# PrimeIntellect-ai/protocol

Measured on AMD Instinct MI355X. Metric: task x worker pair-evals/sec (full-swarm match), higher is better.
Workload: dtype u64

## Files before the change

protocol_amd/csrc/pm_device.h:

```cpp
#ifndef PM_DEVICE_H
#define PM_DEVICE_H

#include <hip/hip_runtime.h>
#include <stdint.h>

#include "pm_engine.h"

namespace pm {

static constexpr double PM_RAD = 3.14159265358979323846 / 180.0;
static constexpr uint64_t PM_KEY_NOLOC = 0x7FEFFFFFFFFFFFFFull;
static constexpr double PM_A_MAX_SAFE = 1.0 - 1.0 / 1048576.0;
static constexpr double PM_A_CHORD_MIN = 1.3e-6;
static constexpr uint32_t PM_CARVE_SLOTS = 8192;
static constexpr uint32_t PM_CARVE_PART = 64;
static constexpr uint32_t PM_CARVE_SEL_CAP = 256;
static constexpr uint32_t PM_CARVE_SLOT_BITS = 13;
static constexpr uint32_t PM_CARVE_BIG_SLOTS = 262144;
static constexpr uint32_t PM_CARVE_SLOT_BITS_BIG = 18;
static constexpr uint32_t PM_CARVE_SLOT_BITS_MEM = 21;
static constexpr double PM_TIE_BAND = 1.0 / 68719476736.0;
static constexpr double PM_TIE_BAND_BIG = 1.0 / 2147483648.0;
static constexpr double PM_TIE_BAND_MEM = 1.0 / 268435456.0;
static constexpr uint32_t PM_PROP_ROW = 96;
// ... 85 lines not shown
  const uint32_t* t_prefix;
  pm_assignment* table;
  uint32_t* task_col;
  pm_assignment* h_table;
  uint32_t* h_gtask;
};

struct MatchPrepArgs {
  uint32_t W, G;
  const int32_t* group_of;
  const uint32_t *g_cfg, *g_n, *g_off, *members, *addr_rank, *g_task;
  uint64_t* sel;
  uint32_t *first, *count;
  uint32_t *rank_in_group, *by_rank;
  uint32_t* g_task_next;
};

struct RowUpdateArgs {
  uint32_t n;
  const double *lat_in, *lon_in;
  const uint32_t* u32_in;
  uint32_t *flags, *gpu_count, *gpu_mem, *gpu_cls, *cpu_cores, *ram, *storage, *addr_rank, *site;
  double *lat, *lon, *coslat;
  double *ux, *uy, *uz;
};

enum { CARVE_MODE_FORM = 0, CARVE_MODE_MERGE = 1 };
enum { CARVE_STATE_RUNNING = 0, CARVE_STATE_DONE = 1, CARVE_STATE_UNCERTAIN = 2, CARVE_STATE_OVERFLOW = 3,
       CARVE_STATE_ABORTED = 4 };
enum {
// ... 143 lines not shown
void launch_explain(const CompatArgs& p, const uint32_t* rows, uint32_t n, uint32_t stride, uint32_t* why_out, hipStream_t s);
void launch_config_report(const ReportArgs& a, uint32_t max_blocks, hipStream_t s);
void launch_task_report(const ReportArgs& a, uint32_t max_blocks, hipStream_t s);
void launch_geo(const double* lat, const double* lon, double* coslat, double* ux, double* uy, double* uz, uint32_t W,
                hipStream_t s);
void launch_triad(const double* b, const double* c, double* a, size_t n, hipStream_t s);
#ifdef PM_ROW_BENCH
hipError_t launch_row_bench(const CarveArgs* d_args, uint32_t seed, uint32_t ci, uint32_t reps, uint32_t mode, unsigned long long* d_out, hipStream_t s);
#endif
void launch_row_network_test(const uint64_t* keys, const uint32_t* sites, uint32_t n_waves, uint32_t n_per_wave, uint32_t slot_bits,
                             uint64_t ulps, uint32_t upto, uint64_t* rows_out, uint32_t* mismatches, hipStream_t s);
static constexpr uint32_t PM_DK_WORDS = 20;
void launch_distance_key_test(const double* in, const double* geo, uint32_t n, uint32_t mode, double* out, hipStream_t s);
void launch_update_rows(const RowUpdateArgs& a, hipStream_t s);
void launch_worker_selector(const int32_t* group_of, const uint32_t* g_cfg, uint32_t R, const uint32_t* rows,
                            uint64_t* sel, hipStream_t s);
void launch_eligible_selector(const uint32_t* wflags, const int32_t* group_of, const uint64_t* compat,
                              uint64_t enabled, uint32_t W, const uint8_t* shard, uint32_t my_rank, uint64_t* sel,
                              hipStream_t s);
void launch_chooser_rank(const int32_t* group_of, const uint64_t* g_id, const uint32_t* count, uint32_t R,
                         const uint32_t* rows, uint64_t seed, uint32_t* rank, hipStream_t s);
void launch_table_scatter(const pm_assignment* x, const uint32_t* xrow, uint32_t W, pm_assignment* table,
                          uint32_t* task_col, uint32_t* g_task_next, const uint64_t* t_live, const uint32_t* t_prefix,
                          hipStream_t s);
void launch_group_rank(const int32_t* group_of, const uint32_t* g_n, const uint32_t* g_off, const uint32_t* members,
                       const uint32_t* addr_rank, uint32_t W, uint32_t* rank_in_group, uint32_t* by_rank,
                       hipStream_t s);
void launch_claim_publish(const ClaimArgs& a, hipStream_t s);
void launch_match_prep(const MatchPrepArgs& a, hipStream_t s);
void launch_build_planes(const uint64_t* col_mask, uint32_t n_cols, uint32_t c_begin, uint32_t c_end, uint32_t stride,
                         uint32_t n_planes, uint64_t* planes, hipStream_t s);
void launch_pair_sweep(int variant, const uint64_t* row_sel, uint32_t R, const uint64_t* col_mask,
                       const uint64_t* planes, uint32_t c_begin, uint32_t c_end, uint32_t stride, uint32_t n_planes,
                       uint32_t* first, uint32_t* count, hipStream_t s, bool inited = false);
void launch_pair_select(int variant, const uint64_t* row_sel, uint32_t R, const uint64_t* col_mask,
                        const uint64_t* planes, uint32_t c_begin, uint32_t c_end, uint32_t stride, uint32_t n_planes,
                        const uint32_t* rank, uint32_t* out, hipStream_t s);
void launch_task_prefix(const uint64_t* live, uint32_t w_begin, uint32_t w_end, uint32_t* prefix, hipStream_t s);
void launch_task_delete(const uint32_t* slots, uint32_t n, uint64_t* tmask, uint64_t* live, uint64_t* planes,
                        uint32_t stride, uint32_t n_planes, hipStream_t s);
void launch_task_intern(const uint64_t* tmask, const uint64_t* live, uint32_t u_begin, uint32_t u_end, uint64_t valid,
                        uint64_t* keys, uint32_t n_slots, uint32_t* vals, uint32_t* counter_and_overflow, uint64_t* umask,
                        uint32_t cap_u, hipStream_t s);
void launch_task_compact_class(const uint32_t* first_c, const uint32_t* count_c, const uint64_t* tmask, uint64_t valid,
// ... 26 lines not shown
```

protocol_amd/csrc/pm_engine.cpp:

```cpp
#include <hip/hip_runtime.h>

#include <algorithm>
#include <atomic>
#include <cmath>
#include <chrono>
#include <cstdio>
#include <cstdlib>
#include <cstring>
#include <functional>
#include <memory>
#include <mutex>
#include <string>
#include <thread>
#include <unordered_map>
#include <vector>

#include "pm_device.h"
#include "pm_engine.h"
#include "pm_internal.h"
#include "pm_members.h"

namespace pm {

static thread_local std::string g_last_error;
// ... 123 lines not shown
  *out = e;
  return PM_OK;
}

void pm_engine_destroy(pm_engine* e) {
  if (!e) return;
  (void)hipSetDevice(e->cfg.device);
  (void)hipStreamSynchronize(e->stream);
  e->d_cfgs.release(); e->d_alts.release(); e->d_model_bits.release();
  e->d_flags.release(); e->d_gpu_count.release(); e->d_gpu_mem.release(); e->d_gpu_cls.release();
  e->d_cpu_cores.release(); e->d_ram.release(); e->d_storage.release(); e->d_addr_rank.release();
  e->d_lat.release(); e->d_lon.release(); e->d_coslat.release(); e->d_compat.release();
  e->d_ux.release(); e->d_uy.release(); e->d_uz.release();
  for (int k = 0; k < 3; ++k) { e->d_c_u[k].release(); e->d_cc_u[k].release(); }
  e->d_tmask.release(); e->d_tplanes.release(); e->d_created.release(); e->d_tlive.release(); e->d_tprefix.release();
  e->d_first_c.release(); e->d_count_c.release(); e->d_tdel.release();
  e->d_group_of.release(); e->d_g_cfg.release(); e->d_g_n.release(); e->d_g_off.release();
  e->d_g_task.release(); e->d_g_task_next.release(); e->d_members.release(); e->d_by_rank.release();
  e->d_rank_in_group.release(); e->d_g_id.release();
  e->d_order.release(); e->d_c_lat.release(); e->d_c_lon.release(); e->d_c_cos.release();
  e->d_cc_lat.release(); e->d_cc_lon.release(); e->d_cc_cos.release(); e->d_slot_pos.release(); e->d_slot_wid.release();
  e->d_site.release(); e->d_c_site.release(); e->d_cc_site.release(); e->d_prop.release(); e->d_prop_send.release(); e->d_seed_map.release(); e->d_seed_prefix.release(); e->d_seed_slots.release(); e->d_prep_block_counts.release(); e->d_prep_counts.release();
  e->d_c_compat.release(); e->d_keys.release(); e->d_bits.release(); e->d_status.release(); e->d_carve_args.release();
  e->d_m_cfg.release(); e->d_m_n.release(); e->d_m_off.release(); e->d_m_members.release();
  e->d_cfgbits.release(); e->d_stream_sq.release(); e->d_stream_row_lo.release(); e->d_stream_row_hi.release();
  e->d_stream_ctl.release(); e->d_stream_trace.release();
  e->d_sel.release(); e->d_wplanes.release(); e->d_sel_perm.release();
  e->d_first.release(); e->d_count.release(); e->d_rank.release(); e->d_chosen.release(); e->d_perm.release();
  e->d_table.release(); e->d_task_col.release(); e->d_shard.release(); e->d_own_rows.release(); e->d_xrow.release();
  e->d_sel_own.release(); e->d_table_x.release(); e->d_row_stage.release(); if (e->h_row_pin) (void)hipHostFree(e->h_row_pin); if (e->ev_row_stage) (void)hipEventDestroy(e->ev_row_stage); e->d_nb_idx.release(); e->d_nb_val.release();
  if (e->h_gstage) (void)hipHostFree(e->h_gstage);
// ... 39 lines not shown
  }
  std::lock_guard<std::mutex> lk(e->mu);
  if (e->dist_phase != 0) return set_error(PM_ESTATE, "a stepwise tick is in progress");
  HIPCHK(hipSetDevice(e->cfg.device));
  e->cfgs.assign(cfgs, cfgs + n_cfgs);
  e->alts.assign(alts, alts + n_alts);
  int32_t rc = upload(e->d_cfgs, e->cfgs.data(), e->cfgs.size(), e->stream);
  if (rc) return rc;
  rc = upload(e->d_alts, e->alts.data(), e->alts.size(), e->stream);
  if (rc) return rc;
  HIPCHK(e->d_model_bits.ensure(1));
  HIPCHK(hipStreamSynchronize(e->stream));
  e->have_cfgs = true;
  e->compat_dirty = true;
  e->tplanes_dirty = true;
  return PM_OK;
}

int32_t pm_set_model_table(pm_engine* e, const uint32_t* bits, uint32_t n_rows, uint32_t n_classes) {
  if (!e || (n_rows && n_classes && !bits)) return set_error(PM_EINVAL, "null argument");
  std::lock_guard<std::mutex> lk(e->mu);
  HIPCHK(hipSetDevice(e->cfg.device));
  const size_t words = size_t(n_rows) * ((n_classes + 31u) / 32u);
  e->model_bits.assign(bits, bits + words);
  e->model_rows = n_rows;
  e->model_classes = n_classes;
  e->cls_check_dirty = true;
  int32_t rc = upload(e->d_model_bits, e->model_bits.data(), words, e->stream);
  if (rc) return rc;
  HIPCHK(hipStreamSynchronize(e->stream));
// ... 22 lines not shown
```

protocol_amd/csrc/pm_engine_match.inc:

```

static int32_t ensure_task_planes(pm_engine* e) {
  if (!e->have_tasks) return set_error(PM_ESTATE, "tasks must be uploaded first");
  const uint32_t n_planes = uint32_t(e->cfgs.size());
  const uint32_t stride = e->t_cap / 64u;
  if (e->tplanes_dirty) {
    HIPCHK(e->d_tplanes.ensure(std::max<size_t>(size_t(stride) * (n_planes + 1), 1)));
    launch_build_planes(e->d_tmask.p, e->t_cap, e->t_lo, e->t_cap, stride, n_planes, e->d_tplanes.p, e->stream);
    HIPCHK(hipGetLastError());
    e->tplanes_dirty = false;
  }
  if (e->tprefix_dirty) {
    launch_task_prefix(e->d_tlive.p, e->t_lo / 64u, stride, e->d_tprefix.p, e->stream);
    HIPCHK(hipGetLastError());
    e->tprefix_dirty = false;
  }
  return PM_OK;
}

static uint32_t task_position(pm_engine* e, uint32_t u) {
  if (u == PM_NONE || u < e->t_lo || u >= e->t_cap) return PM_NONE;
  if (!e->h_tprefix_valid) {
    const uint32_t stride = e->t_cap / 64u;
    e->h_tprefix.assign(stride, 0);
    uint32_t acc = 0;
    for (uint32_t j = e->t_lo / 64u; j < stride; ++j) {
      e->h_tprefix[j] = acc;
      acc += uint32_t(__builtin_popcountll(e->h_tlive[j]));
    }
    e->h_tprefix_valid = true;
// ... 55 lines not shown
  rc = ensure_task_planes(e);
  if (rc) return rc;
  host_mark("match: task planes");
  const uint32_t R = dist ? uint32_t(e->h_own_rows.size()) : e->W;
  const uint32_t* rows = dist ? e->d_own_rows.p : nullptr;
  rc = ensure_sweep_outputs(e, R);
  if (rc) return rc;
  HIPCHK(e->d_sel.ensure(std::max<uint32_t>(e->W, 1)));
  HIPCHK(e->d_table.ensure(std::max<uint32_t>(e->W, 1)));
  HIPCHK(e->d_task_col.ensure(std::max<uint32_t>(e->W, 1)));
  if (e->W == 0) return PM_OK;
  const uint32_t n_planes = uint32_t(e->cfgs.size());

  host_mark("match: selector launch");
  const size_t G = G_ub ? G_ub : e->d_n_groups;
  if (!dist) {
    MatchPrepArgs m{};
    m.W = e->W;
    m.G = uint32_t(G);
    m.group_of = e->d_group_of.p;
    m.g_cfg = e->d_g_cfg.p;
    m.g_n = e->d_g_n.p;
    m.g_off = e->d_g_off.p;
    m.members = e->d_members.p;
    m.addr_rank = e->d_addr_rank.p;
    m.g_task = e->d_g_task.p;
    m.sel = e->d_sel.p;
    m.first = e->d_first.p;
    m.count = e->d_count.p;
    m.rank_in_group = e->d_rank_in_group.p;
    m.by_rank = e->d_by_rank.p;
    m.g_task_next = e->d_g_task_next.p;
    launch_match_prep(m, e->stream);
  } else {
    launch_worker_selector(e->d_group_of.p, e->d_g_cfg.p, R, rows, e->d_sel.p, e->stream);
  }
  const bool time_sweep = e->cfg.time_proposer != 0;
  if (time_sweep) HIPCHK(hipEventRecord(e->kev[4], e->stream));
  const uint32_t t_stride = e->t_cap / 64u;
  launch_pair_sweep(variant, e->d_sel.p, R, e->d_tmask.p, e->d_tplanes.p, e->t_lo, e->t_cap, t_stride, n_planes,
                    e->d_first.p, e->d_count.p, e->stream, !dist);
  if (time_sweep) HIPCHK(hipEventRecord(e->kev[5], e->stream));
  e->k_sweep_recorded = time_sweep;
  const uint32_t* chosen = e->d_first.p;
  if (e->cfg.chooser == PM_CHOOSE_SEEDED) {
    launch_chooser_rank(e->d_group_of.p, e->d_g_id.p, e->d_count.p, R, rows, e->cfg.chooser_seed, e->d_rank.p,
                        e->stream);
    launch_pair_select(variant, e->d_sel.p, R, e->d_tmask.p, e->d_tplanes.p, e->t_lo, e->t_cap, t_stride, n_planes,
                       e->d_rank.p, e->d_chosen.p, e->stream);
    chosen = e->d_chosen.p;
  }
  if (dist) {
    launch_group_rank(e->d_group_of.p, e->d_g_n.p, e->d_g_off.p, e->d_members.p, e->d_addr_rank.p, e->W,
                      e->d_rank_in_group.p, e->d_by_rank.p, e->stream);
    if (G) HIPCHK(hipMemcpyAsync(e->d_g_task_next.p, e->d_g_task.p, G * 4, hipMemcpyDeviceToDevice, e->stream));
  }
  ClaimArgs c{};
  c.R = R;
  c.rows = rows;
  c.group_of = e->d_group_of.p;
  c.g_n = e->d_g_n.p;
  c.g_off = e->d_g_off.p;
  c.g_task = e->d_g_task.p;
  c.g_id = e->d_g_id.p;
  c.g_task_next = e->d_g_task_next.p;
  c.chosen = chosen;
  c.rank_in_group = e->d_rank_in_group.p;
  c.by_rank = e->d_by_rank.p;
  c.t_live = e->d_tlive.p;
  c.t_prefix = e->d_tprefix.p;
  c.table = dist ? e->d_table_x.p + size_t(e->dist_rank) * e->dist_cap_t : e->d_table.p;
  c.task_col = e->d_task_col.p;
  c.h_table = claim_h_table;
  c.h_gtask = claim_h_gtask;
  launch_claim_publish(c, e->stream);
  HIPCHK(hipGetLastError());
  if (want_count && count_out) {
    count_out->resize(R);
    HIPCHK(hipMemcpyAsync(count_out->data(), e->d_count.p, size_t(R) * 4, hipMemcpyDeviceToHost, e->stream));
  }
  return PM_OK;
}

static int32_t pub_buffer(pm_engine* e, PubTable& t, uint32_t rows, uint64_t** out) {
  uint64_t* words = t.words.load(std::memory_order_relaxed);
  if (t.cap_rows < rows || !words) {
    const size_t cap = std::max<size_t>(size_t(rows) + rows / 8 + 64, 64);
    uint64_t* nw = nullptr;
    if (hipHostMalloc((void**)&nw, cap * 32) != hipSuccess || !nw)
      return set_error(PM_ENOMEM, "out of pinned host memory for the published table");
    std::memset(nw, 0, cap * 32);
// ... 205 lines not shown
```

protocol_amd/csrc/pm_engine_state.inc:

```
struct pm_engine {
  pm_engine_config cfg{};
  hipStream_t stream = nullptr;
  hipStream_t stream_owned = nullptr;
  bool own_stream = true;
  hipEvent_t ev[6]{};
  hipEvent_t kev[6]{};
  hipEvent_t k_carve_begin = nullptr;
  hipEvent_t k_compat_end = nullptr;
  bool one_event_behind_carve = false;
  float k_ms_compat = 0, k_ms_carve = 0, k_ms_sweep = 0;
  bool k_sweep_recorded = false, k_compat_recorded = false;
  std::chrono::steady_clock::time_point tick_t0{};
  bool end_event_queued = false;
  uint64_t tick_cand_sum = 0;
  unsigned long long carve_prof[64]{};
  unsigned long long carve_why[24]{};
  uint32_t debug_mem_above = 0;
  uint32_t debug_abort_after = 0;
  uint32_t delta_pushes = 0;
  uint32_t merge_streamed = 0;
  uint32_t merge_stream_min = 512;
  uint32_t prune_mode = 1;
  uint32_t prune_factor = 512;
  uint32_t walk_cap_div = 0;
// ... 43 lines not shown
  uint32_t t_regrowths = 0, t_compactions = 0;
  bool have_tasks = false;
  std::vector<uint64_t> h_tmask, h_tuid, h_tlive;
  std::vector<int64_t> h_created;
  std::vector<uint32_t> h_tprefix;
  bool h_tprefix_valid = false;
  bool tasks_have_uid = false;
  std::unordered_map<uint64_t, uint32_t> uid_to_u;
  bool uid_map_valid = false;
  uint32_t cfg_app_count[PM_MAX_CONFIGS]{};
  bool cfg_app_valid = false;
  DevBuf<uint64_t> d_tmask, d_tplanes, d_tlive;
  DevBuf<int64_t> d_created;
  DevBuf<uint32_t> d_tprefix, d_first_c, d_count_c, d_tdel;
  bool tplanes_dirty = true, tprefix_dirty = true;

  std::vector<Group> groups;
  size_t n_dead_groups = 0;
  bool flags_dirty = false;
  std::vector<int32_t> h_group_of;
  uint64_t id_rng = 0;
  bool groups_dirty = true;
  bool groups_delta_ok = false;
  std::vector<uint32_t> delta_free;
  uint32_t delta_tail_from = PM_NONE;
  bool flags_delta_ok = false;
  std::vector<uint32_t> delta_flags;
  uint32_t* h_delta_pin[2] = {nullptr, nullptr};
  size_t h_delta_cap[2] = {0, 0};
  DevBuf<uint32_t> d_delta[2];
// ... 83 lines not shown
```

protocol_amd/csrc/pm_engine_tasks.inc:

```
static int32_t tasks_alloc(pm_engine* e, uint32_t cap) {
  e->h_tmask.assign(cap, 0);
  e->h_created.assign(cap, 0);
  e->h_tlive.assign(cap / 64u, 0);
  if (e->tasks_have_uid) e->h_tuid.assign(cap, 0); else e->h_tuid.clear();
  e->t_cap = cap;
  e->t_lo = cap;
  e->T = e->t_dead = 0;
  e->h_tprefix_valid = false;
  HIPCHK(e->d_tmask.ensure(cap));
  HIPCHK(e->d_created.ensure(cap));
  HIPCHK(e->d_tlive.ensure(cap / 64u));
  HIPCHK(e->d_tprefix.ensure(cap / 64u));
  HIPCHK(hipMemsetAsync(e->d_tmask.p, 0, size_t(cap) * 8, e->stream));
  HIPCHK(hipMemsetAsync(e->d_tlive.p, 0, size_t(cap / 64u) * 8, e->stream));
  e->tplanes_dirty = true;
  e->tprefix_dirty = true;
  return PM_OK;
}

static int32_t tasks_push_range(pm_engine* e, uint32_t u0, uint32_t u1) {
  if (u1 <= u0) return PM_OK;
  const uint32_t w0 = u0 / 64u, w1 = (u1 + 63u) / 64u;
  HIPCHK(hipMemcpyAsync(e->d_tmask.p + u0, e->h_tmask.data() + u0, size_t(u1 - u0) * 8, hipMemcpyHostToDevice, e->stream));
  HIPCHK(hipMemcpyAsync(e->d_created.p + u0, e->h_created.data() + u0, size_t(u1 - u0) * 8, hipMemcpyHostToDevice, e->stream));
  HIPCHK(hipMemcpyAsync(e->d_tlive.p + w0, e->h_tlive.data() + w0, size_t(w1 - w0) * 8, hipMemcpyHostToDevice, e->stream));
  return PM_OK;
}

static constexpr uint32_t PM_TASK_DEAD_SLACK = 4096;

static int32_t tasks_rebuild(pm_engine* e, uint32_t cap) {
// ... 62 lines not shown
  for (uint32_t u = clear_from; u < lo; ++u) e->h_tmask[u] = 0;
  for (uint32_t w = clear_from / 64u; w < cap / 64u; ++w) e->h_tlive[w] = 0;
  std::memcpy(e->h_tmask.data() + lo, t->topo_mask, size_t(n) * 8);
  std::memcpy(e->h_created.data() + lo, t->created_at, size_t(n) * 8);
  if (t->uid) std::memcpy(e->h_tuid.data() + lo, t->uid, size_t(n) * 8);
  for (uint32_t u = lo; u < cap; ++u) e->h_tlive[u >> 6] |= 1ull << (u & 63u);
  e->t_lo = lo;
  e->T = n;
  e->t_dead = 0;
  e->h_tprefix_valid = false;
  rc = tasks_push_range(e, clear_from, cap);
  if (rc) return rc;
  HIPCHK(hipStreamSynchronize(e->stream));
  e->tplanes_dirty = true;
  e->tprefix_dirty = true;
  e->have_tasks = true;
  size_t n_claim = 0;
  for (const Group& g : e->groups) n_claim += (!g.dead && g.task != PM_NONE);
  if (n_claim) {
    size_t hcap = 64;
    while (hcap < n_claim * 4) hcap <<= 1;
    const uint64_t EMPTY = ~0ull;
    std::vector<uint64_t> keys(hcap, EMPTY);
    std::vector<uint32_t> vals(hcap, PM_NONE);
    auto slot_of = [&](uint64_t k) {
      size_t h = size_t(splitmix64_mix(k)) & (hcap - 1);
      while (keys[h] != EMPTY && keys[h] != k) h = (h + 1) & (hcap - 1);
      return h;
    };
    if (e->tasks_have_uid) {
// ... 97 lines not shown
      }
    }
  }
  {
    int32_t rcp = tasks_push_range(e, lo, e->t_lo);
    if (rcp) return rcp;
  }
  if (!e->tplanes_dirty && e->d_tplanes.p)
    launch_build_planes(e->d_tmask.p, e->t_cap, lo, e->t_lo, e->t_cap / 64u, uint32_t(e->cfgs.size()), e->d_tplanes.p,
                        e->stream);
  HIPCHK(hipGetLastError());
  HIPCHK(hipStreamSynchronize(e->stream));
  e->t_lo = lo;
  e->T += n;
  e->tprefix_dirty = true;
  e->h_tprefix_valid = false;
  pub_shift_tasks(e, n);
  return PM_OK;
}

int32_t pm_tasks_delete(pm_engine* e, const uint64_t* uids, uint32_t n, uint32_t* n_deleted) {
  if (!e || (n && !uids)) return set_error(PM_EINVAL, "null argument");
  std::lock_guard<std::mutex> lk(e->mu);
  HIPCHK(hipSetDevice(e->cfg.device));
  if (n_deleted) *n_deleted = 0;
  if (!e->have_tasks) return set_error(PM_ESTATE, "tasks must be uploaded first");
  if (!e->tasks_have_uid) return set_error(PM_ESTATE, "the task table carries no ids (pm_task_soa.uid)");
  if (e->dist_phase != 0) return set_error(PM_ESTATE, "a stepwise tick is in progress");
  ABSORB_PENDING(e);
  if (!e->uid_map_valid) {
// ... 35 lines not shown
    e->h_tlive[u >> 6] &= ~(1ull << (u & 63u));
  }
  e->h_tprefix_valid = false;
  for (size_t g = 0; g < e->groups.size(); ++g) {
    const Group& gr = e->groups[g];
    if (!gr.dead && gr.task != PM_NONE && std::binary_search(slots.begin(), slots.end(), gr.task))
      dissolve_locked(e, uint32_t(g));
  }
  e->T -= uint32_t(slots.size());
  e->t_dead += uint32_t(slots.size());
  while (e->t_lo < e->t_cap && !((e->h_tlive[e->t_lo >> 6] >> (e->t_lo & 63u)) & 1ull)) {
    e->t_lo++;
    e->t_dead--;
  }
  e->tprefix_dirty = true;
  e->h_tprefix_valid = false;
  if (e->t_dead > e->T + PM_TASK_DEAD_SLACK) {
    int32_t rc = tasks_rebuild(e, e->t_cap);
    if (rc) return rc;
    e->t_compactions++;
  }
  if (n_deleted) *n_deleted = uint32_t(slots.size());
  pub_patch(e, nullptr);
  return PM_OK;
}
```

protocol_amd/csrc/pm_kernels.hip:

```cpp
#include <hip/hip_runtime.h>
#include <stdint.h>

#include "pm_device.h"

#if defined(__HIP_DEVICE_COMPILE__) && !defined(__gfx950__)
#error "pm_kernels.hip is written for gfx950 (MI355X): see the note on the placement kernels' fences above"
#endif

namespace pm {


template <int CTRL, int ROW_MASK>
__device__ __forceinline__ uint32_t dpp_add_step(uint32_t v) {
  return v + (uint32_t)__builtin_amdgcn_update_dpp(0, (int)v, CTRL, ROW_MASK, 0xF, false);
}
__device__ __forceinline__ uint32_t wave_incl_scan_u32(uint32_t v) {
  v = dpp_add_step<0x111, 0xF>(v);
  v = dpp_add_step<0x112, 0xF>(v);
  v = dpp_add_step<0x114, 0xF>(v);
  v = dpp_add_step<0x118, 0xF>(v);
  v = dpp_add_step<0x142, 0xA>(v);
  v = dpp_add_step<0x143, 0xC>(v);
  return v;
}
// ... 338 lines not shown
  out[r] = res;
}

__global__ __launch_bounds__(64) void task_prefix_kernel(const uint64_t* __restrict__ live, uint32_t w_begin,
                                                         uint32_t w_end, uint32_t* __restrict__ prefix) {
  const uint32_t lane = threadIdx.x;
  uint32_t acc = 0;
  for (uint32_t j0 = w_begin; j0 < w_end; j0 += 64u) {
    const uint32_t j = j0 + lane;
    const uint32_t cnt = j < w_end ? (uint32_t)__popcll(live[j]) : 0u;
    const uint32_t incl = wave_incl_scan_u32(cnt);
    if (j < w_end) prefix[j] = acc + incl - cnt;
    acc += __shfl(incl, 63, 64);
  }
}
__global__ __launch_bounds__(256) void task_delete_kernel(const uint32_t* __restrict__ slots, uint32_t n,
                                                          uint64_t* __restrict__ tmask,
                                                          uint64_t* __restrict__ live, uint64_t* __restrict__ planes,
                                                          uint32_t stride, uint32_t n_planes) {
  const uint32_t k = blockIdx.x * 256u + threadIdx.x;
  if (k >= n) return;
  const uint32_t u = slots[k];
  const uint64_t bit = 1ull << (u & 63u);
  tmask[u] = 0ull;
  atomicAnd((unsigned long long*)&live[u >> 6], ~bit);
  for (uint32_t b = 0; b <= n_planes; ++b)
    atomicAnd((unsigned long long*)&planes[(size_t)b * stride + (u >> 6)], ~bit);
}
__global__ __launch_bounds__(256) void task_compact_kernel(const uint32_t* __restrict__ first_u,
                                                           const uint32_t* __restrict__ count_u, uint32_t u_begin,
// ... 70 lines not shown
  uint32_t first = PM_NONE, count = 0u;
  if (m != 0ull) {
    uint32_t h = (uint32_t)splitmix64_mix(m) & h_mask;
    while (keys[h] != m) h = (h + 1u) & h_mask;
    const uint32_t id = vals[h];
    first = first_c[id];
    count = count_c[id];
  }
  first_out[pos] = first;
  count_out[pos] = count;
}

__global__ __launch_bounds__(256) void worker_selector_kernel(const int32_t* __restrict__ group_of,
                                                              const uint32_t* __restrict__ g_cfg, uint32_t R,
                                                              const uint32_t* __restrict__ rows,
                                                              uint64_t* __restrict__ sel) {
  const uint32_t r = blockIdx.x * 256u + threadIdx.x;
  if (r >= R) return;
  const int32_t g = group_of[rows ? rows[r] : r];
  sel[r] = g >= 0 ? (1ull << g_cfg[g]) : 0ull;
}

__global__ __launch_bounds__(256) void chooser_rank_kernel(const int32_t* __restrict__ group_of,
                                                           const uint64_t* __restrict__ g_id,
                                                           const uint32_t* __restrict__ count, uint32_t R,
                                                           const uint32_t* __restrict__ rows, uint64_t seed,
                                                           uint32_t* __restrict__ rank) {
  const uint32_t r = blockIdx.x * 256u + threadIdx.x;
  if (r >= R) return;
  const int32_t g = group_of[rows ? rows[r] : r];
  const uint32_t n = count[r];
  rank[r] = (g >= 0 && n) ? (uint32_t)(splitmix64_mix(seed ^ g_id[g]) % n) : PM_NONE;
}

__global__ __launch_bounds__(256) void eligible_selector_kernel(const uint32_t* __restrict__ wflags,
// ... 29 lines not shown
  by_rank[off + idx] = w;
}

__global__ __launch_bounds__(256) void match_prep_kernel(MatchPrepArgs p) {
  const uint32_t w = blockIdx.x * 256u + threadIdx.x;
  if (w < p.G) p.g_task_next[w] = p.g_task[w];
  if (w >= p.W) return;
  const int32_t g = p.group_of[w];
  p.first[w] = PM_NONE;
  p.count[w] = 0u;
  if (g < 0) {
    p.sel[w] = 0ull;
    p.rank_in_group[w] = 0;
    return;
  }
  p.sel[w] = 1ull << p.g_cfg[g];
  const uint32_t n = p.g_n[g], off = p.g_off[g], my = p.addr_rank[w];
  uint32_t idx = 0;
  for (uint32_t k = 0; k < n; ++k) idx += p.addr_rank[p.members[off + k]] < my;
  p.rank_in_group[w] = idx;
  p.by_rank[off + idx] = w;
}

__device__ __forceinline__ uint32_t task_position(const uint64_t* __restrict__ live, const uint32_t* __restrict__ prefix,
                                                  uint32_t u) {
  return prefix[u >> 6] + (uint32_t)__popcll(live[u >> 6] & ((1ull << (u & 63u)) - 1ull));
}

__global__ __launch_bounds__(256) void claim_publish_kernel(ClaimArgs p) {
  const uint32_t r = blockIdx.x * 256u + threadIdx.x;
  const bool in = r < p.R;
// ... 33 lines not shown
  }
  if (p.h_table) {
    static_assert(sizeof(pm_assignment) == 32, "a row is two 16-byte pieces");
    __shared__ uint4 s_rows[512];
    s_rows[2u * threadIdx.x] = make_uint4(a.task, a.group_slot, a.group_index, a.group_size);
    s_rows[2u * threadIdx.x + 1u] = make_uint4(a.next_worker, 0u, (uint32_t)a.group_id, (uint32_t)(a.group_id >> 32));
    if (g >= 0 && a.group_index == 0u) p.h_gtask[g] = t;
    __syncthreads();
    const uint32_t row0 = blockIdx.x * 256u;
    const uint32_t n16 = 2u * (p.R - row0 < 256u ? p.R - row0 : 256u);
    uint4* const dst = reinterpret_cast<uint4*>(p.h_table + row0);
    for (uint32_t k = threadIdx.x; k < n16; k += 256u) dst[k] = s_rows[k];
  }
}

__global__ __launch_bounds__(256) void table_scatter_kernel(const pm_assignment* __restrict__ x,
                                                            const uint32_t* __restrict__ xrow, uint32_t W,
                                                            pm_assignment* __restrict__ table,
                                                            uint32_t* __restrict__ task_col,
                                                            uint32_t* __restrict__ g_task_next,
                                                            const uint64_t* __restrict__ t_live,
                                                            const uint32_t* __restrict__ t_prefix) {
  const uint32_t w = blockIdx.x * 256u + threadIdx.x;
  if (w >= W) return;
  pm_assignment a = x[xrow[w]];
  if (a.group_slot != PM_NONE && a.task != PM_NONE) g_task_next[a.group_slot] = a.task;
  if (a.task != PM_NONE) a.task = task_position(t_live, t_prefix, a.task);
  table[w] = a;
  task_col[w] = a.task;
}
// ... 57 lines not shown
```

protocol_amd/csrc/pm_launch.inc:

```

void launch_compat(const CompatArgs& a, hipStream_t s) {
  if (a.W == 0) return;
  if (a.W < 65536u)
    hipLaunchKernelGGL(compat_sliced_kernel, dim3((a.W + 63u) / 64u), dim3(256), 0, s, a);
  else
    hipLaunchKernelGGL(compat_kernel, dim3((a.W + 255u) / 256u), dim3(256), 0, s, a);
}
void launch_triad(const double* b, const double* c, double* a, size_t n, hipStream_t s) {
  hipLaunchKernelGGL(triad_kernel, dim3(256 * 32), dim3(256), 0, s, b, c, a, n);
}
void launch_row_network_test(const uint64_t* keys, const uint32_t* sites, uint32_t n_waves, uint32_t n_per_wave, uint32_t slot_bits,
                             uint64_t ulps, uint32_t upto, uint64_t* rows_out, uint32_t* mismatches, hipStream_t s) {
  hipLaunchKernelGGL(row_network_test_kernel, dim3(n_waves / 4u), dim3(256), 0, s, keys, sites, n_per_wave, slot_bits, ulps, upto, rows_out,
                     mismatches);
}
void launch_distance_key_test(const double* in, const double* geo, uint32_t n, uint32_t mode, double* out, hipStream_t s) {
  if (n == 0) return;
  hipLaunchKernelGGL(distance_key_test_kernel, dim3((n + 255u) / 256u), dim3(256), 0, s, in, geo, n, mode, out);
}
void launch_geo(const double* lat, const double* lon, double* coslat, double* ux, double* uy, double* uz, uint32_t W,
                hipStream_t s) {
  if (W == 0) return;
  hipLaunchKernelGGL(geo_kernel, dim3((W + 255u) / 256u), dim3(256), 0, s, lat, lon, coslat, ux, uy, uz, W);
}
void launch_update_rows(const RowUpdateArgs& a, hipStream_t s) {
  if (a.n == 0) return;
  hipLaunchKernelGGL(update_rows_kernel, dim3((a.n + 255u) / 256u), dim3(256), 0, s, a);
}
void launch_worker_selector(const int32_t* group_of, const uint32_t* g_cfg, uint32_t R, const uint32_t* rows,
                            uint64_t* sel, hipStream_t s) {
  if (R == 0) return;
  hipLaunchKernelGGL(worker_selector_kernel, dim3((R + 255u) / 256u), dim3(256), 0, s, group_of, g_cfg, R, rows, sel);
}
void launch_chooser_rank(const int32_t* group_of, const uint64_t* g_id, const uint32_t* count, uint32_t R,
                         const uint32_t* rows, uint64_t seed, uint32_t* rank, hipStream_t s) {
  if (R == 0) return;
  hipLaunchKernelGGL(chooser_rank_kernel, dim3((R + 255u) / 256u), dim3(256), 0, s, group_of, g_id, count, R, rows,
                     seed, rank);
}
void launch_eligible_selector(const uint32_t* wflags, const int32_t* group_of, const uint64_t* compat,
                              uint64_t enabled, uint32_t W, const uint8_t* shard, uint32_t my_rank, uint64_t* sel,
                              hipStream_t s) {
  if (W == 0) return;
  hipLaunchKernelGGL(eligible_selector_kernel, dim3((W + 255u) / 256u), dim3(256), 0, s, wflags, group_of, compat,
                     enabled, W, shard, my_rank, sel);
}
void launch_table_scatter(const pm_assignment* x, const uint32_t* xrow, uint32_t W, pm_assignment* table,
// ... 2 lines not shown
  if (W == 0) return;
  hipLaunchKernelGGL(table_scatter_kernel, dim3((W + 255u) / 256u), dim3(256), 0, s, x, xrow, W, table, task_col,
                     g_task_next, t_live, t_prefix);
}
void launch_group_rank(const int32_t* group_of, const uint32_t* g_n, const uint32_t* g_off, const uint32_t* members,
                       const uint32_t* addr_rank, uint32_t W, uint32_t* rank_in_group, uint32_t* by_rank,
                       hipStream_t s) {
  if (W == 0) return;
  hipLaunchKernelGGL(group_rank_kernel, dim3((W + 255u) / 256u), dim3(256), 0, s, group_of, g_n, g_off, members,
                     addr_rank, W, rank_in_group, by_rank);
}
void launch_match_prep(const MatchPrepArgs& a, hipStream_t s) {
  const uint32_t n = a.W > a.G ? a.W : a.G;
  if (n == 0) return;
  hipLaunchKernelGGL(match_prep_kernel, dim3((n + 255u) / 256u), dim3(256), 0, s, a);
}
void launch_claim_publish(const ClaimArgs& a, hipStream_t s) {
  if (a.R == 0) return;
  hipLaunchKernelGGL(claim_publish_kernel, dim3((a.R + 255u) / 256u), dim3(256), 0, s, a);
}

void launch_build_planes(const uint64_t* col_mask, uint32_t n_cols, uint32_t c_begin, uint32_t c_end, uint32_t stride,
                         uint32_t n_planes, uint64_t* planes, hipStream_t s) {
  const uint32_t w0 = c_begin / 64u, w1 = (c_end + 63u) / 64u;
  if (w1 <= w0) return;
  hipLaunchKernelGGL(build_planes_kernel, dim3(((w1 - w0) * 64u + 255u) / 256u), dim3(256), 0, s, col_mask, n_cols, w0,
                     w1, stride, n_planes, planes);
}

void launch_pair_sweep(int variant, const uint64_t* row_sel, uint32_t R, const uint64_t* col_mask,
// ... 213 lines not shown
```

Measured before the change: 1048 billion.

## Precompute per-config task summaries and fuse match prep with claim publish

Adds a plane-summary kernel that computes, for each config plane, the first eligible task and the count of eligible tasks. It is recomputed only when the task set changes. Because each worker's selector is a single config bit, the per-worker pair sweep reduces to a table lookup and is skipped for non-legacy variants. In the non-distributed, unseeded case, a new fused match_publish kernel replaces the prep, sweep and claim kernels, cutting launches and redundant passes. The risks are extra invalidation bookkeeping (tsum_dirty) and a possible semantic mismatch if selectors ever carry more than one config bit.

```diff
diff --git a/protocol_amd/csrc/pm_device.h b/protocol_amd/csrc/pm_device.h
--- a/protocol_amd/csrc/pm_device.h
+++ b/protocol_amd/csrc/pm_device.h
@@ -123,6 +123,24 @@
   uint32_t *first, *count;
   uint32_t *rank_in_group, *by_rank;
   uint32_t* g_task_next;
+  const uint32_t *tsum_first, *tsum_count;
+};
+
+struct MatchPublishArgs {
+  uint32_t W, G;
+  uint32_t members_cap;
+  const int32_t* group_of;
+  const uint32_t *g_cfg, *g_n, *g_off, *members, *addr_rank, *g_task;
+  const uint64_t* g_id;
+  const uint32_t *tsum_first, *tsum_count;
+  const uint64_t* t_live;
+  const uint32_t* t_prefix;
+  uint32_t* g_task_next;
+  uint32_t* count_out;
+  pm_assignment* table;
+  uint32_t* task_col;
+  pm_assignment* h_table;
+  uint32_t* h_gtask;
 };
 
 struct RowUpdateArgs {
@@ -296,7 +314,8 @@
 void launch_distance_key_test(const double* in, const double* geo, uint32_t n, uint32_t mode, double* out, hipStream_t s);
 void launch_update_rows(const RowUpdateArgs& a, hipStream_t s);
 void launch_worker_selector(const int32_t* group_of, const uint32_t* g_cfg, uint32_t R, const uint32_t* rows,
-                            uint64_t* sel, hipStream_t s);
+                            uint64_t* sel, const uint32_t* tsum_first, const uint32_t* tsum_count, uint32_t* first,
+                            uint32_t* count, hipStream_t s);
 void launch_eligible_selector(const uint32_t* wflags, const int32_t* group_of, const uint64_t* compat,
                               uint64_t enabled, uint32_t W, const uint8_t* shard, uint32_t my_rank, uint64_t* sel,
                               hipStream_t s);
@@ -310,6 +329,9 @@
                        hipStream_t s);
 void launch_claim_publish(const ClaimArgs& a, hipStream_t s);
 void launch_match_prep(const MatchPrepArgs& a, hipStream_t s);
+void launch_match_publish(const MatchPublishArgs& a, hipStream_t s);
+void launch_plane_summary(const uint64_t* planes, uint32_t stride, uint32_t w_begin, uint32_t w_end, uint32_t n_planes,
+                          uint32_t* tsum_first, uint32_t* tsum_count, hipStream_t s);
 void launch_build_planes(const uint64_t* col_mask, uint32_t n_cols, uint32_t c_begin, uint32_t c_end, uint32_t stride,
                          uint32_t n_planes, uint64_t* planes, hipStream_t s);
 void launch_pair_sweep(int variant, const uint64_t* row_sel, uint32_t R, const uint64_t* col_mask,
diff --git a/protocol_amd/csrc/pm_engine.cpp b/protocol_amd/csrc/pm_engine.cpp
--- a/protocol_amd/csrc/pm_engine.cpp
+++ b/protocol_amd/csrc/pm_engine.cpp
@@ -161,7 +161,7 @@
   e->d_ux.release(); e->d_uy.release(); e->d_uz.release();
   for (int k = 0; k < 3; ++k) { e->d_c_u[k].release(); e->d_cc_u[k].release(); }
   e->d_tmask.release(); e->d_tplanes.release(); e->d_created.release(); e->d_tlive.release(); e->d_tprefix.release();
-  e->d_first_c.release(); e->d_count_c.release(); e->d_tdel.release();
+  e->d_first_c.release(); e->d_count_c.release(); e->d_tdel.release(); e->d_tsum.release();
   e->d_group_of.release(); e->d_g_cfg.release(); e->d_g_n.release(); e->d_g_off.release();
   e->d_g_task.release(); e->d_g_task_next.release(); e->d_members.release(); e->d_by_rank.release();
   e->d_rank_in_group.release(); e->d_g_id.release();
@@ -231,6 +231,7 @@
   e->have_cfgs = true;
   e->compat_dirty = true;
   e->tplanes_dirty = true;
+  e->tsum_dirty = true;
   return PM_OK;
 }
 
diff --git a/protocol_amd/csrc/pm_engine_match.inc b/protocol_amd/csrc/pm_engine_match.inc
--- a/protocol_amd/csrc/pm_engine_match.inc
+++ b/protocol_amd/csrc/pm_engine_match.inc
@@ -8,11 +8,25 @@
     launch_build_planes(e->d_tmask.p, e->t_cap, e->t_lo, e->t_cap, stride, n_planes, e->d_tplanes.p, e->stream);
     HIPCHK(hipGetLastError());
     e->tplanes_dirty = false;
+    e->tsum_dirty = true;
   }
   if (e->tprefix_dirty) {
     launch_task_prefix(e->d_tlive.p, e->t_lo / 64u, stride, e->d_tprefix.p, e->stream);
     HIPCHK(hipGetLastError());
     e->tprefix_dirty = false;
+  }
+  if (e->tsum_dirty) {
+    HIPCHK(e->d_tsum.ensure(2u * PM_MAX_CONFIGS));
+    const bool timed = e->cfg.time_proposer != 0 && e->cfg.sweep_variant != 1u;
+    if (timed) HIPCHK(hipEventRecord(e->kev[4], e->stream));
+    launch_plane_summary(e->d_tplanes.p, stride, e->t_lo / 64u, stride, n_planes, e->d_tsum.p, e->d_tsum.p + PM_MAX_CONFIGS,
+                         e->stream);
+    HIPCHK(hipGetLastError());
+    if (timed) {
+      HIPCHK(hipEventRecord(e->kev[5], e->stream));
+      e->k_sweep_recorded = true;
+    }
+    e->tsum_dirty = false;
   }
   return PM_OK;
 }
@@ -98,10 +112,14 @@
 
   host_mark("match: selector launch");
   const size_t G = G_ub ? G_ub : e->d_n_groups;
-  if (!dist) {
-    MatchPrepArgs m{};
+  const bool summary = variant != 1;
+  const uint32_t* const tsum_first = summary ? e->d_tsum.p : nullptr;
+  const uint32_t* const tsum_count = summary ? e->d_tsum.p + PM_MAX_CONFIGS : nullptr;
+  if (summary && !dist && e->cfg.chooser != PM_CHOOSE_SEEDED) {
+    MatchPublishArgs m{};
     m.W = e->W;
-    m.G = uint32_t(G);
+    m.G = uint32_t(std::min(G, std::min(e->d_g_cfg.cap, std::min(e->d_g_n.cap, e->d_g_off.cap))));
+    m.members_cap = uint32_t(std::min<size_t>(e->d_members.cap, 0xFFFFFFFFu));
     m.group_of = e->d_group_of.p;
     m.g_cfg = e->d_g_cfg.p;
     m.g_n = e->d_g_n.p;
@@ -109,56 +127,87 @@
     m.members = e->d_members.p;
     m.addr_rank = e->d_addr_rank.p;
     m.g_task = e->d_g_task.p;
-    m.sel = e->d_sel.p;
-    m.first = e->d_first.p;
-    m.count = e->d_count.p;
-    m.rank_in_group = e->d_rank_in_group.p;
-    m.by_rank = e->d_by_rank.p;
+    m.g_id = e->d_g_id.p;
+    m.tsum_first = tsum_first;
+    m.tsum_count = tsum_count;
+    m.t_live = e->d_tlive.p;
+    m.t_prefix = e->d_tprefix.p;
     m.g_task_next = e->d_g_task_next.p;
-    launch_match_prep(m, e->stream);
+    m.count_out = want_count && count_out ? e->d_count.p : nullptr;
+    m.table = e->d_table.p;
+    m.task_col = e->d_task_col.p;
+    m.h_table = claim_h_table;
+    m.h_gtask = claim_h_gtask;
+    launch_match_publish(m, e->stream);
+    HIPCHK(hipGetLastError());
   } else {
-    launch_worker_selector(e->d_group_of.p, e->d_g_cfg.p, R, rows, e->d_sel.p, e->stream);
-  }
-  const bool time_sweep = e->cfg.time_proposer != 0;
-  if (time_sweep) HIPCHK(hipEventRecord(e->kev[4], e->stream));
-  const uint32_t t_stride = e->t_cap / 64u;
-  launch_pair_sweep(variant, e->d_sel.p, R, e->d_tmask.p, e->d_tplanes.p, e->t_lo, e->t_cap, t_stride, n_planes,
-                    e->d_first.p, e->d_count.p, e->stream, !dist);
-  if (time_sweep) HIPCHK(hipEventRecord(e->kev[5], e->stream));
-  e->k_sweep_recorded = time_sweep;
-  const uint32_t* chosen = e->d_first.p;
-  if (e->cfg.chooser == PM_CHOOSE_SEEDED) {
-    launch_chooser_rank(e->d_group_of.p, e->d_g_id.p, e->d_count.p, R, rows, e->cfg.chooser_seed, e->d_rank.p,
-                        e->stream);
-    launch_pair_select(variant, e->d_sel.p, R, e->d_tmask.p, e->d_tplanes.p, e->t_lo, e->t_cap, t_stride, n_planes,
-                       e->d_rank.p, e->d_chosen.p, e->stream);
-    chosen = e->d_chosen.p;
-  }
-  if (dist) {
-    launch_group_rank(e->d_group_of.p, e->d_g_n.p, e->d_g_off.p, e->d_members.p, e->d_addr_rank.p, e->W,
-                      e->d_rank_in_group.p, e->d_by_rank.p, e->stream);
-    if (G) HIPCHK(hipMemcpyAsync(e->d_g_task_next.p, e->d_g_task.p, G * 4, hipMemcpyDeviceToDevice, e->stream));
-  }
-  ClaimArgs c{};
-  c.R = R;
-  c.rows = rows;
-  c.group_of = e->d_group_of.p;
-  c.g_n = e->d_g_n.p;
-  c.g_off = e->d_g_off.p;
-  c.g_task = e->d_g_task.p;
-  c.g_id = e->d_g_id.p;
-  c.g_task_next = e->d_g_task_next.p;
-  c.chosen = chosen;
-  c.rank_in_group = e->d_rank_in_group.p;
-  c.by_rank = e->d_by_rank.p;
-  c.t_live = e->d_tlive.p;
-  c.t_prefix = e->d_tprefix.p;
-  c.table = dist ? e->d_table_x.p + size_t(e->dist_rank) * e->dist_cap_t : e->d_table.p;
-  c.task_col = e->d_task_col.p;
-  c.h_table = claim_h_table;
-  c.h_gtask = claim_h_gtask;
-  launch_claim_publish(c, e->stream);
-  HIPCHK(hipGetLastError());
+    if (!dist) {
+      MatchPrepArgs m{};
+      m.W = e->W;
+      m.G = uint32_t(G);
+      m.group_of = e->d_group_of.p;
+      m.g_cfg = e->d_g_cfg.p;
+      m.g_n = e->d_g_n.p;
+      m.g_off = e->d_g_off.p;
+      m.members = e->d_members.p;
+      m.addr_rank = e->d_addr_rank.p;
+      m.g_task = e->d_g_task.p;
+      m.sel = e->d_sel.p;
+      m.first = e->d_first.p;
+      m.count = e->d_count.p;
+      m.rank_in_group = e->d_rank_in_group.p;
+      m.by_rank = e->d_by_rank.p;
+      m.g_task_next = e->d_g_task_next.p;
+      m.tsum_first = tsum_first;
+      m.tsum_count = tsum_count;
+      launch_match_prep(m, e->stream);
+    } else {
+      launch_worker_selector(e->d_group_of.p, e->d_g_cfg.p, R, rows, e->d_sel.p, tsum_first, tsum_count, e->d_first.p,
+                             e->d_count.p, e->stream);
+    }
+    const uint32_t t_stride = e->t_cap / 64u;
+    if (!summary) {
+      const bool time_sweep = e->cfg.time_proposer != 0;
+      if (time_sweep) HIPCHK(hipEventRecord(e->kev[4], e->stream));
+      launch_pair_sweep(variant, e->d_sel.p, R, e->d_tmask.p, e->d_tplanes.p, e->t_lo, e->t_cap, t_stride, n_planes,
+                        e->d_first.p, e->d_count.p, e->stream, !dist);
+      if (time_sweep) HIPCHK(hipEventRecord(e->kev[5], e->stream));
+      e->k_sweep_recorded = time_sweep;
+    }
+    const uint32_t* chosen = e->d_first.p;
+    if (e->cfg.chooser == PM_CHOOSE_SEEDED) {
+      launch_chooser_rank(e->d_group_of.p, e->d_g_id.p, e->d_count.p, R, rows, e->cfg.chooser_seed, e->d_rank.p,
+                          e->stream);
+      launch_pair_select(variant, e->d_sel.p, R, e->d_tmask.p, e->d_tplanes.p, e->t_lo, e->t_cap, t_stride, n_planes,
+                         e->d_rank.p, e->d_chosen.p, e->stream);
+      chosen = e->d_chosen.p;
+    }
+    if (dist) {
+      launch_group_rank(e->d_group_of.p, e->d_g_n.p, e->d_g_off.p, e->d_members.p, e->d_addr_rank.p, e->W,
+                        e->d_rank_in_group.p, e->d_by_rank.p, e->stream);
+      if (G) HIPCHK(hipMemcpyAsync(e->d_g_task_next.p, e->d_g_task.p, G * 4, hipMemcpyDeviceToDevice, e->stream));
+    }
+    ClaimArgs c{};
+    c.R = R;
+    c.rows = rows;
+    c.group_of = e->d_group_of.p;
+    c.g_n = e->d_g_n.p;
+    c.g_off = e->d_g_off.p;
+    c.g_task = e->d_g_task.p;
+    c.g_id = e->d_g_id.p;
+    c.g_task_next = e->d_g_task_next.p;
+    c.chosen = chosen;
+    c.rank_in_group = e->d_rank_in_group.p;
+    c.by_rank = e->d_by_rank.p;
+    c.t_live = e->d_tlive.p;
+    c.t_prefix = e->d_tprefix.p;
+    c.table = dist ? e->d_table_x.p + size_t(e->dist_rank) * e->dist_cap_t : e->d_table.p;
+    c.task_col = e->d_task_col.p;
+    c.h_table = claim_h_table;
+    c.h_gtask = claim_h_gtask;
+    launch_claim_publish(c, e->stream);
+    HIPCHK(hipGetLastError());
+  }
   if (want_count && count_out) {
     count_out->resize(R);
     HIPCHK(hipMemcpyAsync(count_out->data(), e->d_count.p, size_t(R) * 4, hipMemcpyDeviceToHost, e->stream));
diff --git a/protocol_amd/csrc/pm_engine_state.inc b/protocol_amd/csrc/pm_engine_state.inc
--- a/protocol_amd/csrc/pm_engine_state.inc
+++ b/protocol_amd/csrc/pm_engine_state.inc
@@ -81,6 +81,8 @@
   DevBuf<int64_t> d_created;
   DevBuf<uint32_t> d_tprefix, d_first_c, d_count_c, d_tdel;
   bool tplanes_dirty = true, tprefix_dirty = true;
+  DevBuf<uint32_t> d_tsum;
+  bool tsum_dirty = true;
 
   std::vector<Group> groups;
   size_t n_dead_groups = 0;
diff --git a/protocol_amd/csrc/pm_engine_tasks.inc b/protocol_amd/csrc/pm_engine_tasks.inc
--- a/protocol_amd/csrc/pm_engine_tasks.inc
+++ b/protocol_amd/csrc/pm_engine_tasks.inc
@@ -15,6 +15,7 @@
   HIPCHK(hipMemsetAsync(e->d_tlive.p, 0, size_t(cap / 64u) * 8, e->stream));
   e->tplanes_dirty = true;
   e->tprefix_dirty = true;
+  e->tsum_dirty = true;
   return PM_OK;
 }
 
@@ -107,6 +108,7 @@
   HIPCHK(hipStreamSynchronize(e->stream));
   e->tplanes_dirty = true;
   e->tprefix_dirty = true;
+  e->tsum_dirty = true;
   e->have_tasks = true;
   size_t n_claim = 0;
   for (const Group& g : e->groups) n_claim += (!g.dead && g.task != PM_NONE);
@@ -234,6 +236,7 @@
   e->t_lo = lo;
   e->T += n;
   e->tprefix_dirty = true;
+  e->tsum_dirty = true;
   e->h_tprefix_valid = false;
   pub_shift_tasks(e, n);
   return PM_OK;
@@ -299,6 +302,7 @@
     e->t_dead--;
   }
   e->tprefix_dirty = true;
+  e->tsum_dirty = true;
   e->h_tprefix_valid = false;
   if (e->t_dead > e->T + PM_TASK_DEAD_SLACK) {
     int32_t rc = tasks_rebuild(e, e->t_cap);
diff --git a/protocol_amd/csrc/pm_kernels.hip b/protocol_amd/csrc/pm_kernels.hip
--- a/protocol_amd/csrc/pm_kernels.hip
+++ b/protocol_amd/csrc/pm_kernels.hip
@@ -376,6 +376,43 @@
     acc += __shfl(incl, 63, 64);
   }
 }
+__global__ __launch_bounds__(256) void plane_summary_kernel(const uint64_t* __restrict__ planes, uint32_t stride,
+                                                            uint32_t w_begin, uint32_t w_end, uint32_t n_planes,
+                                                            uint32_t* __restrict__ tsum_first,
+                                                            uint32_t* __restrict__ tsum_count) {
+  __shared__ uint32_t s_first[4], s_cnt[4];
+  const uint32_t b = blockIdx.x;
+  uint32_t first = PM_NONE, cnt = 0;
+  if (b < n_planes) {
+    const uint64_t* __restrict__ pl = planes + (size_t)b * stride;
+    uint32_t j = w_begin + threadIdx.x;
+    for (; j + 768u < w_end; j += 1024u) {
+      const uint64_t h0 = pl[j], h1 = pl[j + 256u], h2 = pl[j + 512u], h3 = pl[j + 768u];
+      if (first == PM_NONE && (h0 | h1 | h2 | h3)) {
+        const uint32_t u = h0 ? 0u : (h1 ? 1u : (h2 ? 2u : 3u));
+        const uint64_t h = h0 ? h0 : (h1 ? h1 : (h2 ? h2 : h3));
+        first = (j + u * 256u) * 64u + (uint32_t)__builtin_ctzll(h);
+      }
+      cnt += __popcll(h0) + __popcll(h1) + __popcll(h2) + __popcll(h3);
+    }
+    for (; j < w_end; j += 256u) {
+      const uint64_t h = pl[j];
+      if (h && first == PM_NONE) first = j * 64u + (uint32_t)__builtin_ctzll(h);
+      cnt += __popcll(h);
+    }
+  }
+  first = wave_min(first);
+  cnt = wave_sum(cnt);
+  if ((threadIdx.x & 63u) == 0u) {
+    s_first[threadIdx.x >> 6] = first;
+    s_cnt[threadIdx.x >> 6] = cnt;
+  }
+  __syncthreads();
+  if (threadIdx.x == 0u) {
+    tsum_first[b] = min(min(s_first[0], s_first[1]), min(s_first[2], s_first[3]));
+    tsum_count[b] = s_cnt[0] + s_cnt[1] + s_cnt[2] + s_cnt[3];
+  }
+}
 __global__ __launch_bounds__(256) void task_delete_kernel(const uint32_t* __restrict__ slots, uint32_t n,
                                                           uint64_t* __restrict__ tmask,
                                                           uint64_t* __restrict__ live, uint64_t* __restrict__ planes,
@@ -476,11 +513,20 @@
 __global__ __launch_bounds__(256) void worker_selector_kernel(const int32_t* __restrict__ group_of,
                                                               const uint32_t* __restrict__ g_cfg, uint32_t R,
                                                               const uint32_t* __restrict__ rows,
-                                                              uint64_t* __restrict__ sel) {
+                                                              uint64_t* __restrict__ sel,
+                                                              const uint32_t* __restrict__ tsum_first,
+                                                              const uint32_t* __restrict__ tsum_count,
+                                                              uint32_t* __restrict__ first,
+                                                              uint32_t* __restrict__ count) {
   const uint32_t r = blockIdx.x * 256u + threadIdx.x;
   if (r >= R) return;
   const int32_t g = group_of[rows ? rows[r] : r];
-  sel[r] = g >= 0 ? (1ull << g_cfg[g]) : 0ull;
+  const uint32_t cfg = g >= 0 ? g_cfg[g] : 0u;
+  sel[r] = g >= 0 ? (1ull << cfg) : 0ull;
+  if (tsum_first) {
+    first[r] = g >= 0 ? tsum_first[cfg] : PM_NONE;
+    count[r] = g >= 0 ? tsum_count[cfg] : 0u;
+  }
 }
 
 __global__ __launch_bounds__(256) void chooser_rank_kernel(const int32_t* __restrict__ group_of,
@@ -540,7 +586,12 @@
     p.rank_in_group[w] = 0;
     return;
   }
-  p.sel[w] = 1ull << p.g_cfg[g];
+  const uint32_t cfg = p.g_cfg[g];
+  p.sel[w] = 1ull << cfg;
+  if (p.tsum_first) {
+    p.first[w] = p.tsum_first[cfg];
+    p.count[w] = p.tsum_count[cfg];
+  }
   const uint32_t n = p.g_n[g], off = p.g_off[g], my = p.addr_rank[w];
   uint32_t idx = 0;
   for (uint32_t k = 0; k < n; ++k) idx += p.addr_rank[p.members[off + k]] < my;
@@ -604,6 +655,74 @@
   }
 }
 
+__global__ __launch_bounds__(256) void match_publish_kernel(MatchPublishArgs p) {
+  const uint32_t w = blockIdx.x * 256u + threadIdx.x;
+  if (w < p.G) {
+    uint32_t t = p.g_task[w];
+    const uint32_t off = p.g_off[w];
+    bool named = false;
+    if (p.g_n[w] != 0u && off < p.members_cap) {
+      const uint32_t m = p.members[off];
+      named = m < p.W && p.group_of[m] == (int32_t)w;
+    }
+    if (t == PM_NONE && named) t = p.tsum_first[p.g_cfg[w]];
+    p.g_task_next[w] = t;
+    if (p.h_gtask && named) p.h_gtask[w] = t;
+  }
+  const bool in = w < p.W;
+  const int32_t g = in ? p.group_of[w] : -1;
+  pm_assignment a;
+  a.task = PM_NONE;
+  a.group_slot = PM_NONE;
+  a.group_index = 0;
+  a.group_size = 0;
+  a.next_worker = PM_NONE;
+  a.group_id = 0;
+  uint32_t cnt = 0u;
+  if (g >= 0) {
+    const uint32_t cfg = p.g_cfg[g];
+    uint32_t t = p.g_task[g];
+    if (t == PM_NONE) t = p.tsum_first[cfg];
+    cnt = p.tsum_count[cfg];
+    const uint32_t n = p.g_n[g], off = p.g_off[g], my = p.addr_rank[w];
+    uint32_t idx = 0u, succ = PM_NONE, succ_rank = 0u, lowest = w, lowest_rank = my;
+    for (uint32_t k = 0; k < n; ++k) {
+      const uint32_t m = p.members[off + k];
+      const uint32_t r = p.addr_rank[m];
+      idx += r < my;
+      if (r > my && (succ == PM_NONE || r < succ_rank)) {
+        succ = m;
+        succ_rank = r;
+      }
+      if (r < lowest_rank) {
+        lowest = m;
+        lowest_rank = r;
+      }
+    }
+    a.task = t == PM_NONE ? t : task_position(p.t_live, p.t_prefix, t);
+    a.group_slot = (uint32_t)g;
+    a.group_index = idx;
+    a.group_size = n;
+    a.next_worker = succ != PM_NONE ? succ : lowest;
+    a.group_id = p.g_id[g];
+  }
+  if (in) {
+    p.table[w] = a;
+    p.task_col[w] = a.task;
+    if (p.count_out) p.count_out[w] = cnt;
+  }
+  const uint32_t row0 = blockIdx.x * 256u;
+  if (p.h_table && row0 < p.W) {
+    __shared__ uint4 s_rows[512];
+    s_rows[2u * threadIdx.x] = make_uint4(a.task, a.group_slot, a.group_index, a.group_size);
+    s_rows[2u * threadIdx.x + 1u] = make_uint4(a.next_worker, 0u, (uint32_t)a.group_id, (uint32_t)(a.group_id >> 32));
+    __syncthreads();
+    const uint32_t n16 = 2u * (p.W - row0 < 256u ? p.W - row0 : 256u);
+    uint4* const dst = reinterpret_cast<uint4*>(p.h_table + row0);
+    for (uint32_t k = threadIdx.x; k < n16; k += 256u) dst[k] = s_rows[k];
+  }
+}
+
 __global__ __launch_bounds__(256) void table_scatter_kernel(const pm_assignment* __restrict__ x,
                                                             const uint32_t* __restrict__ xrow, uint32_t W,
                                                             pm_assignment* __restrict__ table,
diff --git a/protocol_amd/csrc/pm_launch.inc b/protocol_amd/csrc/pm_launch.inc
--- a/protocol_amd/csrc/pm_launch.inc
+++ b/protocol_amd/csrc/pm_launch.inc
@@ -28,9 +28,11 @@
   hipLaunchKernelGGL(update_rows_kernel, dim3((a.n + 255u) / 256u), dim3(256), 0, s, a);
 }
 void launch_worker_selector(const int32_t* group_of, const uint32_t* g_cfg, uint32_t R, const uint32_t* rows,
-                            uint64_t* sel, hipStream_t s) {
+                            uint64_t* sel, const uint32_t* tsum_first, const uint32_t* tsum_count, uint32_t* first,
+                            uint32_t* count, hipStream_t s) {
   if (R == 0) return;
-  hipLaunchKernelGGL(worker_selector_kernel, dim3((R + 255u) / 256u), dim3(256), 0, s, group_of, g_cfg, R, rows, sel);
+  hipLaunchKernelGGL(worker_selector_kernel, dim3((R + 255u) / 256u), dim3(256), 0, s, group_of, g_cfg, R, rows, sel,
+                     tsum_first, tsum_count, first, count);
 }
 void launch_chooser_rank(const int32_t* group_of, const uint64_t* g_id, const uint32_t* count, uint32_t R,
                          const uint32_t* rows, uint64_t seed, uint32_t* rank, hipStream_t s) {
@@ -63,6 +65,16 @@
   const uint32_t n = a.W > a.G ? a.W : a.G;
   if (n == 0) return;
   hipLaunchKernelGGL(match_prep_kernel, dim3((n + 255u) / 256u), dim3(256), 0, s, a);
+}
+void launch_match_publish(const MatchPublishArgs& a, hipStream_t s) {
+  const uint32_t n = a.W > a.G ? a.W : a.G;
+  if (n == 0) return;
+  hipLaunchKernelGGL(match_publish_kernel, dim3((n + 255u) / 256u), dim3(256), 0, s, a);
+}
+void launch_plane_summary(const uint64_t* planes, uint32_t stride, uint32_t w_begin, uint32_t w_end, uint32_t n_planes,
+                          uint32_t* tsum_first, uint32_t* tsum_count, hipStream_t s) {
+  hipLaunchKernelGGL(plane_summary_kernel, dim3(PM_MAX_CONFIGS), dim3(256), 0, s, planes, stride, w_begin, w_end, n_planes,
+                     tsum_first, tsum_count);
 }
 void launch_claim_publish(const ClaimArgs& a, hipStream_t s) {
   if (a.R == 0) return;
```

Result: no change. 1047 billion (-0.1%).
